# leeyevi/MV3D_TF

Measured on AMD Instinct MI355X. Metric: KITTI-shape frames/sec (RPN+3-view ROI-pool+NMS) at 1/2/4/8 MI355X, higher is better.
Workload: dtype f32

## Files before the change

### include/mv3d_hip.h

```cpp
#ifndef MV3D_HIP_H
#define MV3D_HIP_H
#include <stddef.h>
#include <stdint.h>
#ifdef __cplusplus
extern "C" {
#endif

typedef enum {
    MV3D_OK = 0,
    MV3D_ERR_INVALID_ARG = 1,
    MV3D_ERR_WORKSPACE = 2,
    MV3D_ERR_HIP = 3,
    MV3D_ERR_ZERO_DIVISION = 4
} mv3d_status;

int mv3d_version(void);
const char *mv3d_status_string(int status);


size_t mv3d_nms_workspace_bytes(int max_boxes);
int mv3d_nms_device(const float *dets_dev, int n, double thresh, int max_keep,
                    int32_t *keep_dev, int32_t *num_keep_dev, int32_t *status_dev,
                    void *workspace, size_t workspace_bytes, void *stream);

// ... 158 lines not shown
int mv3d_proposal_target_stage2_batch_devn(int batch, const float *const *rois_bv_dev, const float *const *rois_3d_dev,
                                           const int *num_rois_cap, const int32_t *const *num_rois_dev,
                                           const float *const *gt_bv_dev, const float *const *gt_3d_dev,
                                           const float *const *gt_corners_dev, const int *G, const float *const *calib_dev,
                                           const mv3d_proposal_target_params *params, const int32_t *const *fg_pick_dev,
                                           const int *n_fg, const int32_t *const *bg_pick_dev, const int *n_bg,
                                           float *const *rois_bv_out, float *const *rois_img_out, int32_t *const *labels_out,
                                           float *const *bbox_targets_out, float *const *rois_3d_out, float *const *rois_fv_out,
                                           void *const *workspace, const size_t *workspace_bytes, void *stream);

int mv3d_point_cloud_2_top(const float *points_dev, int num_points, float *top_dev, void *stream);

int mv3d_point_cloud_2_top_shape(double res, double zres, double side_lo, double side_hi, double fwd_lo, double fwd_hi,
                                 double height_lo, double height_hi, int *dims);
int mv3d_point_cloud_2_top_ranges(const float *points_dev, int num_points, double res, double zres, double side_lo, double side_hi,
                                  double fwd_lo, double fwd_hi, double height_lo, double height_hi, float *top_dev,
                                  int *status_dev, void *stream);

int mv3d_legacy_permutation(void *mt19937_state, int32_t n, int32_t *out);
typedef struct {
    int32_t n_fg, n_bg, n_low;
    int32_t pt_n_fg, pt_n_bg;
    int32_t reserved0;
    const uint8_t *fg_alive;
} mv3d_draw_frame;
typedef struct {
    int32_t rpn_batchsize;
    int32_t rpn_num_fg;
    int32_t rois_per_image;
    int32_t roi_fg_max;
} mv3d_draw_params;
int mv3d_draw_training_subsamples(void *mt19937_state, int batch, const mv3d_draw_frame *frames, const mv3d_draw_params *par,
                                  int32_t *lists, size_t lists_cap, int32_t *sizes, int32_t *scratch, size_t scratch_cap);

typedef struct {
    int32_t batch, H, W, num_classes;
    int32_t proposal_cap;
    int32_t anchor_cap;
    int32_t roi_cap;
    int32_t max_gt;
    mv3d_proposal_params proposal;
    mv3d_anchor_target_params anchor;
    mv3d_proposal_target_params target;
    mv3d_draw_params draw;
} mv3d_train_path_config;
typedef struct {
    float *blob_bv, *blob_img, *blob_3d;
    int32_t *num_proposals;
    void *proposal_ws; size_t proposal_ws_bytes;
    float *rpn_labels, *rpn_targets;
    float *anchors, *anchors_3d;
    int32_t *n_anchors;
    uint8_t *report; size_t report_row;
    int32_t *pt_counts;
    void *anchor_ws; size_t anchor_ws_bytes;
    void *target_ws; size_t target_ws_bytes;
    float *rois_bev, *rois_rgb, *rois_fv;
    float *rois_3d; int32_t *labels; float *bbox_targets;
    int32_t *lists; size_t lists_cap;
    uint8_t *h_report; size_t h_report_row;
    int32_t *h_pt_counts;
    int32_t *h_num_proposals;
    int32_t *h_lists;
    int32_t *h_scratch; size_t scratch_cap;
} mv3d_train_path_slot;
typedef struct mv3d_train_path mv3d_train_path;
int mv3d_train_path_create(const mv3d_train_path_config *config, int depth, const mv3d_train_path_slot *slots, int helper_thread,
                           mv3d_train_path **out);
int mv3d_train_path_configure(mv3d_train_path *path, const mv3d_train_path_config *config);
int mv3d_train_path_submit(mv3d_train_path *path, int slot, const float *prob_dev, const float *pred_dev, const float *im_info_dev,
                           const float *calib_dev, const float *const *gt_bv_dev, const float *const *gt_3d_dev,
                           const float *const *gt_corners_dev, const int *G, void *mt19937_state, void *stream);
int mv3d_train_path_finish(mv3d_train_path *path, int slot, int32_t *rows_out, int32_t *num_proposals_out, int32_t *sizes_out);
int mv3d_train_path_host_seconds(mv3d_train_path *path, double *wait_s, double *draw_s);
void mv3d_train_path_destroy(mv3d_train_path *path);

int mv3d_gt_encode(const float *box_cam_dev, const double *cos_sin_dev, int num_objects, const float *inv_rot_dev,
                   const float *tr_velo_to_cam_dev, float *corners_cam_dev, float *corners_lidar_dev,
                   float *boxes_3d_dev, float *boxes_bv_dev, void *stream);

int mv3d_box_detect_tail(const float *rois_3d_dev, const float *bbox_pred_dev, int num_rois, int num_classes,
                         float *corners_dev, float *pred_cnr_r_dev, float *pred_bv_dev, float *pred_bv_r_dev,
                         void *stream);

typedef struct {
    int32_t num_classes;
    int32_t rows_per_frame;
    int32_t max_per_image;
    int32_t nms_strict_gt;
    float score_thresh;
    int32_t reserved0;
    double nms_thresh;
} mv3d_detect_post_params;

size_t mv3d_detect_post_workspace_bytes(int batch, const mv3d_detect_post_params *p);
int mv3d_detect_post(const float *cls_prob_dev, const float *pred_bv_dev, const float *corners_dev,
                     const float *pred_cnr_r_dev, const int32_t *num_rois_dev, int batch,
                     const mv3d_detect_post_params *p, float *det_bv_dev, float *det_cnr_dev, float *det_cnr_r_dev,
                     int32_t *det_row_dev, int32_t *det_count_dev, int32_t *status_dev, void *workspace,
                     size_t workspace_bytes, void *stream);

size_t mv3d_loss_workspace_bytes(int rows);
int mv3d_rpn_loss(const float *rpn_cls_score_dev, const float *rpn_labels_dev, const float *rpn_bbox_pred_dev,
                  const float *rpn_bbox_targets_dev, int num_anchors, float sigma, float *losses_dev,
                  float *d_cls_score_dev, float *d_bbox_pred_dev, void *workspace, size_t workspace_bytes, void *stream);
int mv3d_rcnn_loss(const float *cls_score_dev, const int32_t *labels_dev, const float *bbox_pred_dev,
                   const float *bbox_targets_dev, int num_rois, int num_classes, int box_dim, float sigma,
// ... 167 lines not shown
```

### mv3d_tf_amd/_lib.py

```python
import ctypes as C
import os

import torch

_HERE = os.path.dirname(os.path.abspath(__file__))
LIB_PATH = os.path.join(_HERE, "libmv3d_hip.so")

OK, ERR_INVALID_ARG, ERR_WORKSPACE, ERR_HIP, ERR_ZERO_DIVISION = 0, 1, 2, 3, 4


class ProposalParams(C.Structure):
    _fields_ = [("feat_stride", C.c_int32), ("pre_nms_topN", C.c_int32), ("post_nms_topN", C.c_int32),
                ("img_height", C.c_int32), ("img_width", C.c_int32), ("img_padding", C.c_int32),
                ("nms_strict_gt", C.c_int32), ("reserved0", C.c_int32), ("nms_thresh", C.c_double), ("min_size", C.c_double)]


class DetectPostParams(C.Structure):
    _fields_ = [("num_classes", C.c_int32), ("rows_per_frame", C.c_int32), ("max_per_image", C.c_int32),
                ("nms_strict_gt", C.c_int32), ("score_thresh", C.c_float), ("reserved0", C.c_int32), ("nms_thresh", C.c_double)]


class AnchorTargetParams(C.Structure):
    _fields_ = [("feat_stride", C.c_int32), ("clobber_positives", C.c_int32),
                ("negative_overlap", C.c_double), ("positive_overlap", C.c_double)]
# ... 127 lines not shown
    "mv3d_proposal_target_stage1_batch_devn": (C.c_int, [C.c_int, _P, _P, _P, _P, _P, _P, _P, _P, _P, _P, _P, _P]),
    "mv3d_proposal_target_stage2_batch_devn": (C.c_int, [C.c_int, _P, _P, _P, _P, _P, _P, _P, _P, _P, _P, _P, _P, _P, _P, _P, _P, _P, _P,
                                                         _P, _P, _P, _P, _P]),
    "mv3d_proposal_target_workspace_bytes": (C.c_size_t, [C.c_int, C.c_int]),
    "mv3d_proposal_target_stage1": (C.c_int, [_P, _P, C.c_int, _P, _P, C.c_int, C.POINTER(ProposalTargetParams), _P, _P,
                                              C.c_size_t, _P]),
    "mv3d_proposal_target_stage2": (C.c_int, [_P, _P, C.c_int, _P, _P, _P, C.c_int, _P, C.POINTER(ProposalTargetParams),
                                              _P, C.c_int, _P, C.c_int, _P, _P, _P, _P, _P, _P, C.c_size_t, _P]),
    "mv3d_point_cloud_2_top": (C.c_int, [_P, C.c_int, _P, _P]),
    "mv3d_point_cloud_2_top_shape": (C.c_int, [C.c_double] * 8 + [_P]),
    "mv3d_point_cloud_2_top_ranges": (C.c_int, [_P, C.c_int] + [C.c_double] * 8 + [_P, _P, _P]),
    "mv3d_box_detect_tail": (C.c_int, [_P, _P, C.c_int, C.c_int, _P, _P, _P, _P, _P]),
    "mv3d_detect_post_workspace_bytes": (C.c_size_t, [C.c_int, C.POINTER(DetectPostParams)]),
    "mv3d_detect_post": (C.c_int, [_P, _P, _P, _P, _P, C.c_int, C.POINTER(DetectPostParams), _P, _P, _P, _P, _P, _P, _P, C.c_size_t,
                                   _P]),
    "mv3d_loss_workspace_bytes": (C.c_size_t, [C.c_int]),
    "mv3d_rpn_loss": (C.c_int, [_P, _P, _P, _P, C.c_int, C.c_float, _P, _P, _P, _P, C.c_size_t, _P]),
    "mv3d_rcnn_loss": (C.c_int, [_P, _P, _P, _P, C.c_int, C.c_int, C.c_int, C.c_float, _P, _P, _P, _P, C.c_size_t, _P]),
    "mv3d_roi_pool_forward_views": (C.c_int, [C.c_int, C.POINTER(RoiView), C.c_int, C.c_int, _P]),
    "mv3d_roi_pool_forward_views_cold": (C.c_int, [C.c_int, C.POINTER(RoiView), C.c_int, C.c_int, _P]),
    "mv3d_roi_pool_forward_views_half": (C.c_int, [C.c_int, C.POINTER(RoiView), C.c_int, C.c_int, C.c_int, C.c_int, _P]),
    "mv3d_roi_pool_backward_workspace_bytes": (C.c_size_t, [C.c_int, C.POINTER(RoiGradView), C.c_int, C.c_int]),
    "mv3d_roi_pool_backward_views": (C.c_int, [C.c_int, C.POINTER(RoiGradView), C.c_int, C.c_int, _P, C.c_size_t, _P]),
    "mv3d_roi_pool_pair_workspace_bytes": (C.c_size_t, [C.c_int, C.POINTER(RoiGradView), C.c_int, C.c_int]),
    "mv3d_roi_pool_forward_views_pair": (C.c_int, [C.c_int, C.POINTER(RoiView), C.c_int, C.c_int, C.c_int, _P]),
    "mv3d_roi_pool_backward_views_pair": (C.c_int, [C.c_int, C.POINTER(RoiGradView), C.c_int, C.c_int, _P, C.c_size_t, _P]),
    "mv3d_roi_pool_argmax_decode": (C.c_int, [C.c_int, C.POINTER(RoiView), C.c_int, C.c_int, C.POINTER(C.c_void_p), _P]),
    "mv3d_ROIPoolForwardLaucher": (C.c_int, [_P, C.c_float, C.c_int, C.c_int, C.c_int, C.c_int, C.c_int, C.c_int, _P, _P, _P, _P]),
    "mv3d_ROIPoolBackwardLaucher": (C.c_int, [_P, C.c_float, C.c_int, C.c_int, C.c_int, C.c_int, C.c_int, C.c_int, C.c_int, _P, _P, _P, _P]),
    "mv3d_rois_3d_to_fv": (C.c_int, [_P, C.c_int, _P, _P]),
    "mv3d_legacy_permutation": (C.c_int, [_P, C.c_int32, _P]),
    "mv3d_draw_training_subsamples": (C.c_int, [_P, C.c_int, C.POINTER(DrawFrame), C.POINTER(DrawParams), _P, C.c_size_t, _P, _P,
                                                C.c_size_t]),
    "mv3d_train_path_create": (C.c_int, [C.POINTER(TrainPathConfig), C.c_int, C.POINTER(TrainPathSlot), C.c_int, C.POINTER(C.c_void_p)]),
    "mv3d_train_path_configure": (C.c_int, [_P, C.POINTER(TrainPathConfig)]),
    "mv3d_train_path_submit": (C.c_int, [_P, C.c_int, _P, _P, _P, _P, _P, _P, _P, _P, _P, _P]),
    "mv3d_train_path_finish": (C.c_int, [_P, C.c_int, _P, _P, _P]),
    "mv3d_train_path_host_seconds": (C.c_int, [_P, C.POINTER(C.c_double), C.POINTER(C.c_double)]),
    "mv3d_train_path_destroy": (None, [_P]),
    "mv3d_gt_encode": (C.c_int, [_P, _P, C.c_int, _P, _P, _P, _P, _P, _P, _P]),
    "mv3d_conv3x3_f16": (C.c_int, [_P, _P, _P, _P, C.c_int, C.c_int, C.c_int, C.c_int, C.c_int, C.c_int, C.c_int, C.c_int, _P]),
    "mv3d_conv3x3_f32": (C.c_int, [_P, _P, _P, _P, C.c_int, C.c_int, C.c_int, C.c_int, C.c_int, C.c_int, C.c_int, _P]),
    "mv3d_maxpool2x2_f32": (C.c_int, [_P, _P, C.c_int, C.c_int, C.c_int, C.c_int, _P]),
    "mv3d_frame_nhwc_f32": (C.c_int, [_P, _P, C.c_int, C.c_int, C.c_int, C.c_int, C.c_int, _P]),
    "mv3d_conv3x3_bf16": (C.c_int, [_P, _P, _P, _P, C.c_int, C.c_int, C.c_int, C.c_int, C.c_int, C.c_int, C.c_int, C.c_int, _P]),
    "mv3d_maxpool2x2_bf16": (C.c_int, [_P, _P, C.c_int, C.c_int, C.c_int, C.c_int, _P]),
    "mv3d_frame_nhwc_bf16": (C.c_int, [_P, _P, C.c_int, C.c_int, C.c_int, C.c_int, C.c_int, _P]),
    "mv3d_conv3x3_wgrad_workspace_bytes": (C.c_size_t, [C.c_int, C.c_int, C.c_int, C.c_int, C.c_int]),
    "mv3d_conv3x3_wgrad_bf16": (C.c_int, [_P, _P, _P, _P, C.c_int, C.c_int, C.c_int, C.c_int, C.c_int, C.c_int, _P, C.c_size_t, _P]),
    "mv3d_conv3x3_wgrad_f32_workspace_bytes": (C.c_size_t, [C.c_int, C.c_int, C.c_int, C.c_int, C.c_int]),
    "mv3d_conv3x3_wgrad_f32": (C.c_int, [_P, _P, _P, _P, C.c_int, C.c_int, C.c_int, C.c_int, C.c_int, C.c_int, _P, C.c_size_t, _P]),
    "mv3d_conv3x3_pack_bf16": (C.c_int, [_P, _P, _P, C.c_int, C.c_int, C.c_int, _P]),
    "mv3d_conv3x3_gated_bf16": (C.c_int, [_P, _P, _P, _P, _P, C.c_int, C.c_int, C.c_int, C.c_int, C.c_int, _P]),
    "mv3d_maxpool2x2_bwd_f32": (C.c_int, [_P, _P, _P, C.c_int, C.c_int, C.c_int, C.c_int, _P]),
    "mv3d_maxpool2x2_bwd_bf16": (C.c_int, [_P, _P, _P, C.c_int, C.c_int, C.c_int, C.c_int, _P]),
    "mv3d_conv3x3_views_f16": (C.c_int, [C.c_int, C.POINTER(ConvView), C.c_int, C.c_int, C.c_int, C.c_int, C.c_int, _P]),
    "mv3d_conv3x3_views_bf16": (C.c_int, [C.c_int, C.POINTER(ConvView), C.c_int, C.c_int, C.c_int, C.c_int, C.c_int, _P]),
    "mv3d_conv3x3_views_f32": (C.c_int, [C.c_int, C.POINTER(ConvView), C.c_int, C.c_int, C.c_int, C.c_int, _P]),
    "mv3d_conv3x3_pool_views_f16": (C.c_int, [C.c_int, C.POINTER(ConvView), C.c_int, C.c_int, _P]),
    "mv3d_conv3x3_pool_views_bf16": (C.c_int, [C.c_int, C.POINTER(ConvView), C.c_int, C.c_int, _P]),
    "mv3d_maxpool2x2_views_f16": (C.c_int, [C.c_int, C.POINTER(PoolView), C.c_int, _P]),
    "mv3d_maxpool2x2_views_bf16": (C.c_int, [C.c_int, C.POINTER(PoolView), C.c_int, _P]),
    "mv3d_maxpool2x2_views_f32": (C.c_int, [C.c_int, C.POINTER(PoolView), C.c_int, _P]),
    "mv3d_maxpool2x2_bwd_views_bf16": (C.c_int, [C.c_int, C.POINTER(PoolView), C.c_int, _P]),
    "mv3d_maxpool2x2_bwd_views_f32": (C.c_int, [C.c_int, C.POINTER(PoolView), C.c_int, _P]),
    "mv3d_conv3x3_wgrad_views_workspace_bytes": (C.c_size_t, [C.c_int, C.POINTER(WgradView), C.c_int, C.c_int, C.c_int]),
    "mv3d_conv3x3_wgrad_views_bf16": (C.c_int, [C.c_int, C.POINTER(WgradView), C.c_int, C.c_int, C.c_int, _P, C.c_size_t, _P]),
    "mv3d_conv3x3_wgrad_views_f32": (C.c_int, [C.c_int, C.POINTER(WgradView), C.c_int, C.c_int, C.c_int, _P, C.c_size_t, _P]),
    "mv3d_conv3x3_pack_many_bf16": (C.c_int, [C.c_int, C.POINTER(PackItem), _P]),
    "mv3d_conv3x3_pack_many_f32": (C.c_int, [C.c_int, C.POINTER(PackItem), _P]),
    "mv3d_maxpool2x2_f16": (C.c_int, [_P, _P, C.c_int, C.c_int, C.c_int, C.c_int, _P]),
# ... 51 lines not shown
```

### mv3d_tf_amd/csrc/legacy_rng.hip

```cpp
#include <stdint.h>
#include <string.h>
#include "../../include/mv3d_hip.h"

namespace {

constexpr int MT_N = 624, MT_M = 397;
struct MtState { uint32_t key[MT_N]; int pos; };

inline void mt_gen(MtState *s)
{
    uint32_t *k = s->key;
    int i;
    for (i = 0; i < MT_N - MT_M; ++i) {
        const uint32_t y = (k[i] & 0x80000000u) | (k[i + 1] & 0x7fffffffu);
        k[i] = k[i + MT_M] ^ (y >> 1) ^ ((y & 1u) ? 0x9908b0dfu : 0u);
    }
    for (; i < MT_N - 1; ++i) {
        const uint32_t y = (k[i] & 0x80000000u) | (k[i + 1] & 0x7fffffffu);
        k[i] = k[i + (MT_M - MT_N)] ^ (y >> 1) ^ ((y & 1u) ? 0x9908b0dfu : 0u);
    }
    const uint32_t y = (k[MT_N - 1] & 0x80000000u) | (k[0] & 0x7fffffffu);
    k[MT_N - 1] = k[MT_M - 1] ^ (y >> 1) ^ ((y & 1u) ? 0x9908b0dfu : 0u);
    s->pos = 0;
}

inline uint32_t mt_next(MtState *s)
{
    if (s->pos == MT_N) mt_gen(s);
    uint32_t y = s->key[s->pos++];
    y ^= (y >> 11);
    y ^= (y << 7) & 0x9d2c5680u;
    y ^= (y << 15) & 0xefc60000u;
    y ^= (y >> 18);
    return y;
}

void permutation(MtState *s, int32_t n, int32_t *x)
{
    for (int32_t i = 0; i < n; ++i) x[i] = i;
    int32_t i = n - 1;
    int pos = s->pos;
    uint32_t t[MT_N];
    int t_lo = MT_N;
    while (i >= 1) {
        const uint32_t mask = 0xffffffffu >> __builtin_clz((uint32_t)i);
        const int32_t lo = (int32_t)(mask >> 1);
        while (i > lo) {
            if (pos == MT_N) { mt_gen(s); pos = 0; t_lo = MT_N; }
            if (t_lo > pos) {
                for (int k = pos; k < MT_N; ++k) {
                    uint32_t y = s->key[k];
                    y ^= (y >> 11);
                    y ^= (y << 7) & 0x9d2c5680u;
                    y ^= (y << 15) & 0xefc60000u;
                    y ^= (y >> 18);
                    t[k] = y;
                }
                t_lo = pos;
            }
            while (pos < MT_N && i > lo) {
                const uint32_t j = t[pos++] & mask;
                const bool ok = j <= (uint32_t)i;
                const uint32_t jj = ok ? j : (uint32_t)i;
                const int32_t a = x[i], b = x[jj];
                x[i] = b; x[jj] = a;
                i -= ok ? 1 : 0;
            }
        }
    }
    s->pos = pos;
}

}

extern "C" int mv3d_legacy_permutation(void *mt19937_state, int32_t n, int32_t *out)
{
    if (!mt19937_state || n < 0 || (n > 0 && !out)) return MV3D_ERR_INVALID_ARG;
    MtState *s = (MtState *)mt19937_state;
    if (s->pos < 0 || s->pos > MT_N) return MV3D_ERR_INVALID_ARG;
    permutation(s, n, out);
    return MV3D_OK;
}

extern "C" int mv3d_draw_training_subsamples(void *mt19937_state, int batch, const mv3d_draw_frame *frames,
                                             const mv3d_draw_params *par, int32_t *lists, size_t lists_cap, int32_t *sizes,
                                             int32_t *scratch, size_t scratch_cap)
{
    if (!mt19937_state || batch <= 0 || !frames || !par || !lists || !sizes || !scratch) return MV3D_ERR_INVALID_ARG;
    MtState *s = (MtState *)mt19937_state;
    if (s->pos < 0 || s->pos > MT_N) return MV3D_ERR_INVALID_ARG;
    size_t o = 0;
    auto emit = [&](int32_t n, int32_t take, bool draw, int32_t *size_out) -> bool {
        *size_out = 0;
        if (!draw) return true;
        if (n < 0 || (size_t)n > scratch_cap || take < 0 || take > n || o + (size_t)take > lists_cap) return false;
        if (take == n) {
            permutation(s, n, lists + o);
        } else {
            permutation(s, n, scratch);
            memcpy(lists + o, scratch, (size_t)take * sizeof(int32_t));
        }
        *size_out = take;
        o += (size_t)take;
        return true;
    };
    for (int b = 0; b < batch; ++b) {
        const mv3d_draw_frame &f = frames[b];
        int32_t *sz = sizes + 5 * b;
        if (f.n_fg < 0 || f.n_bg < 0 || f.n_low < 0 || f.pt_n_fg < 0 || f.pt_n_bg < 0 || (f.n_fg > 0 && !f.fg_alive))
            return MV3D_ERR_INVALID_ARG;
        const int32_t num_fg = par->rpn_num_fg;
        const int32_t *dis_fg = lists + o;
        if (!emit(f.n_fg, f.n_fg - num_fg, f.n_fg > num_fg, &sz[0])) return MV3D_ERR_WORKSPACE;
        const int32_t num_bg = par->rpn_batchsize - (f.n_fg < num_fg ? f.n_fg : num_fg);
        if (!emit(f.n_bg, f.n_bg - num_bg, f.n_bg > num_bg, &sz[1])) return MV3D_ERR_WORKSPACE;
        int32_t n_pos = 0;
        if (f.n_fg > 0) {
            if ((size_t)f.n_fg > scratch_cap) return MV3D_ERR_WORKSPACE;
            uint8_t *alive = (uint8_t *)scratch;
            for (int32_t i = 0; i < f.n_fg; ++i) alive[i] = f.fg_alive[i] ? 1 : 0;
            for (int32_t i = 0; i < sz[0]; ++i) alive[dis_fg[i]] = 0;
            for (int32_t i = 0; i < f.n_fg; ++i) n_pos += alive[i];
        }
        const int32_t num_bg2 = par->rpn_batchsize - n_pos;
        if (!emit(f.n_low, f.n_low - num_bg2, f.n_low > num_bg2, &sz[2])) return MV3D_ERR_WORKSPACE;
        const int32_t fg_n = par->roi_fg_max < f.pt_n_fg ? par->roi_fg_max : f.pt_n_fg;
        if (!emit(f.pt_n_fg, fg_n, f.pt_n_fg > 0, &sz[3])) return MV3D_ERR_WORKSPACE;
        const int32_t bg_room = par->rois_per_image - fg_n;
        const int32_t bg_n = bg_room < f.pt_n_bg ? bg_room : f.pt_n_bg;
        if (!emit(f.pt_n_bg, bg_n < 0 ? 0 : bg_n, f.pt_n_bg > 0, &sz[4])) return MV3D_ERR_WORKSPACE;
    }
    return MV3D_OK;
}
```

### mv3d_tf_amd/csrc/train_stream.hip

```cpp
#include <hip/hip_runtime.h>
#include <chrono>
#include <condition_variable>
#include <deque>
#include <mutex>
#include <new>
#include <thread>
#include <vector>
#include "common.h"
#include "../../include/mv3d_hip.h"

#define TP_MAX_BATCH 16

namespace {

enum SlotState { TP_IDLE = 0, TP_SUBMITTED = 1, TP_STAGED = 2 };

struct Slot {
    mv3d_train_path_slot buf;
    hipEvent_t ev = nullptr;
    int state = TP_IDLE, rc = MV3D_OK;
    hipStream_t stream = nullptr;
    void *mt = nullptr;
    const float *calib = nullptr;
    const float *gt_bv[TP_MAX_BATCH], *gt_3d[TP_MAX_BATCH], *gt_c[TP_MAX_BATCH];
// ... 14 lines not shown
{
#ifdef MV3D_TUNING
    return getenv("MV3D_TRAIN_PATH_COPIES") != nullptr;
#else
    return false;
#endif
}

__global__ __launch_bounds__(256) void tp_report_kernel(const uint8_t *__restrict__ report, size_t report_row, uint8_t *__restrict__ h_report,
                                                        size_t h_row, int B, const int32_t *__restrict__ pt_counts, int32_t *__restrict__ h_pt,
                                                        const int32_t *__restrict__ nump, int32_t *__restrict__ h_nump)
{
    const size_t v = h_row / 16;
    for (size_t i = threadIdx.x; i < (size_t)B * v; i += 256) {
        const size_t b = i / v, j = i - b * v;
        reinterpret_cast<uint4 *>(h_report + b * h_row)[j] = reinterpret_cast<const uint4 *>(report + b * report_row)[j];
    }
    for (int i = threadIdx.x; i < 4 * B; i += 256) h_pt[i] = pt_counts[i];
    for (int i = threadIdx.x; i < 2 * B; i += 256) h_nump[i] = nump[i];
}

}

struct mv3d_train_path {
    mv3d_train_path_config cfg;
    mv3d_proposal_target_params tpar[TP_MAX_BATCH];
    int depth = 0, device = 0;
    std::vector<Slot> slots;
    bool threaded = false, stop = false;
    std::thread helper;
    std::mutex m;
    std::condition_variable cv_work, cv_done;
    std::deque<int> queue;
    double t_wait = 0.0, t_draw = 0.0;
};

namespace {

bool config_ok(const mv3d_train_path_config &c)
{
    return c.batch >= 1 && c.batch <= TP_MAX_BATCH && c.H > 0 && c.W > 0 && c.num_classes >= 1 && c.proposal_cap > 0 && c.anchor_cap > 0 &&
           c.roi_cap > 0 && c.max_gt > 0 && c.draw.rois_per_image <= c.roi_cap;
}

void set_params(mv3d_train_path *tp, const mv3d_train_path_config &c)
{
    tp->cfg = c;
    for (int b = 0; b < c.batch; ++b) {
        tp->tpar[b] = c.target;
        tp->tpar[b].num_classes = c.num_classes;
        tp->tpar[b].frame_index = b;
    }
}

bool slot_ok(const mv3d_train_path_config &c, const mv3d_train_path_slot &s)
{
    const size_t N = (size_t)4 * c.H * c.W, B = (size_t)c.batch;
    if (!s.blob_bv || !s.blob_img || !s.blob_3d || !s.num_proposals || !s.proposal_ws || !s.rpn_labels || !s.rpn_targets || !s.anchors ||
        !s.anchors_3d || !s.n_anchors || !s.report || !s.pt_counts || !s.anchor_ws || !s.target_ws || !s.rois_bev || !s.rois_rgb ||
        !s.rois_3d || !s.labels || !s.bbox_targets || !s.lists || !s.h_report || !s.h_pt_counts || !s.h_num_proposals || !s.h_lists ||
        !s.h_scratch)
        return false;
    if (s.report_row % MV3D_ALIGN || s.report_row < 32 + N || s.h_report_row < 32 || s.h_report_row > s.report_row) return false;
    if (s.anchor_ws_bytes % MV3D_ALIGN || s.target_ws_bytes % MV3D_ALIGN) return false;
    if (s.lists_cap < B * (3 * N + 2 * ((size_t)c.proposal_cap + c.max_gt))) return false;
    if (s.scratch_cap < (N > (size_t)c.proposal_cap + c.max_gt ? N : (size_t)c.proposal_cap + c.max_gt)) return false;
    return true;
// ... 18 lines not shown

#define TP_HIP(expr)                                 \
    do {                                             \
        if ((expr) != hipSuccess) return MV3D_ERR_HIP; \
    } while (0)

int host_stage(mv3d_train_path *tp, Slot &s)
{
    const mv3d_train_path_config &c = tp->cfg;
    const mv3d_train_path_slot &u = s.buf;
    const int B = c.batch, H = c.H, W = c.W;
    const auto t0 = std::chrono::steady_clock::now();
    TP_HIP(hipEventSynchronize(s.ev));
    const auto t1 = std::chrono::steady_clock::now();
    for (int b = 0; b < B; ++b)
        if (u.h_num_proposals[B + b] & MV3D_FLAG_ZERO_DIVISION) return MV3D_ERR_ZERO_DIVISION;
    mv3d_draw_frame fr[TP_MAX_BATCH];
    for (int b = 0; b < B; ++b) {
        const uint8_t *head = u.h_report + (size_t)b * u.h_report_row;
        const int32_t *cnt = (const int32_t *)head;
        fr[b].n_fg = cnt[1]; fr[b].n_bg = cnt[2]; fr[b].n_low = cnt[3];
        fr[b].pt_n_fg = u.h_pt_counts[4 * b + 1]; fr[b].pt_n_bg = u.h_pt_counts[4 * b + 2];
        fr[b].reserved0 = 0;
        if (cnt[1] < 0 || (size_t)cnt[1] > (size_t)4 * H * W) return MV3D_ERR_INVALID_ARG;
        if (32 + (size_t)cnt[1] <= u.h_report_row) {
            fr[b].fg_alive = head + 32;
        } else {
            s.spill[b].resize((size_t)cnt[1]);
            TP_HIP(hipMemcpyAsync(s.spill[b].data(), s.a_fgh[b], (size_t)cnt[1], hipMemcpyDeviceToHost, s.stream));
            TP_HIP(hipStreamSynchronize(s.stream));
            fr[b].fg_alive = s.spill[b].data();
        }
    }
    int rc = mv3d_draw_training_subsamples(s.mt, B, fr, &c.draw, u.h_lists, u.lists_cap, s.sizes, u.h_scratch, u.scratch_cap);
    const auto t2 = std::chrono::steady_clock::now();
    {
        std::lock_guard<std::mutex> g(tp->m);
        tp->t_wait += std::chrono::duration<double>(t1 - t0).count();
        tp->t_draw += std::chrono::duration<double>(t2 - t1).count();
    }
    if (rc != MV3D_OK) return rc;
    size_t off[5 * TP_MAX_BATCH + 1];
    off[0] = 0;
    for (int k = 0; k < 5 * B; ++k) off[k + 1] = off[k] + (size_t)s.sizes[k];
    const int32_t *const lists = u.lists;
    if (off[5 * B]) TP_HIP(hipMemcpyAsync(u.lists, u.h_lists, off[5 * B] * sizeof(int32_t), hipMemcpyHostToDevice, s.stream));
    const int32_t *lst[5][TP_MAX_BATCH];
    int cnt[5][TP_MAX_BATCH];
    for (int b = 0; b < B; ++b)
        for (int k = 0; k < 5; ++k) {
            cnt[k][b] = s.sizes[5 * b + k];
            lst[k][b] = cnt[k][b] ? lists + off[5 * b + k] : nullptr;
        }
    rc = mv3d_anchor_target_stage2_batch(B, H, W, &c.anchor, lst[0], cnt[0], lst[1], cnt[1], lst[2], cnt[2], u.rpn_labels, u.anchors,
                                         u.anchors_3d, u.n_anchors, c.anchor_cap, s.a_ws, u.anchor_ws_bytes, s.stream);
    if (rc != MV3D_OK) return rc;
    float *o_bev[TP_MAX_BATCH], *o_rgb[TP_MAX_BATCH], *o_fv[TP_MAX_BATCH], *o_3d[TP_MAX_BATCH], *o_tg[TP_MAX_BATCH];
    int32_t *o_lab[TP_MAX_BATCH];
    const float *cal[TP_MAX_BATCH];
    size_t row = 0;
    for (int b = 0; b < B; ++b) {
        const int S = cnt[3][b] + cnt[4][b];
        s.rows[b] = S;
        if (row + (size_t)S > (size_t)B * c.roi_cap) return MV3D_ERR_WORKSPACE;
        o_bev[b] = S ? u.rois_bev + row * 5 : nullptr;
        o_rgb[b] = S ? u.rois_rgb + row * 5 : nullptr;
        o_fv[b] = (S && u.rois_fv) ? u.rois_fv + row * 5 : nullptr;
        o_3d[b] = S ? u.rois_3d + row * 7 : nullptr;
        o_lab[b] = S ? u.labels + row : nullptr;
        o_tg[b] = S ? u.bbox_targets + row * 24 * c.num_classes : nullptr;
        cal[b] = s.calib + (size_t)b * 48;
        row += (size_t)S;
    }
    return mv3d_proposal_target_stage2_batch_devn(B, s.p_bv, s.p_3d, s.p_cap, s.p_num, s.gt_bv, s.gt_3d, s.gt_c, s.G, cal, tp->tpar, lst[3],
                                                  cnt[3], lst[4], cnt[4], o_bev, o_rgb, o_lab, o_tg, o_3d, u.rois_fv ? o_fv : nullptr, s.p_ws,
                                                  s.p_wsz, s.stream);
}

int host_stage_noexcept(mv3d_train_path *tp, Slot &s)
{
    try {
        return host_stage(tp, s);
    } catch (...) {
        return MV3D_ERR_WORKSPACE;
    }
}

void helper_main(mv3d_train_path *tp)
{
    (void)hipSetDevice(tp->device);
    for (;;) {
        int k;
        {
            std::unique_lock<std::mutex> g(tp->m);
            tp->cv_work.wait(g, [&] { return tp->stop || !tp->queue.empty(); });
            if (tp->queue.empty()) return;
            k = tp->queue.front();
            tp->queue.pop_front();
        }
        Slot &s = tp->slots[k];
        const int rc = host_stage_noexcept(tp, s);
        {
            std::lock_guard<std::mutex> g(tp->m);
            s.rc = rc;
            s.state = TP_STAGED;
        }
        tp->cv_done.notify_all();
    }
}

}

extern "C" int mv3d_train_path_create(const mv3d_train_path_config *config, int depth, const mv3d_train_path_slot *slots, int helper_thread,
                                      mv3d_train_path **out)
{
    if (!config || !slots || !out || depth < 1 || depth > 64 || !config_ok(*config)) return MV3D_ERR_INVALID_ARG;
    for (int k = 0; k < depth; ++k)
        if (!slot_ok(*config, slots[k])) return MV3D_ERR_INVALID_ARG;
    mv3d_train_path *tp = new (std::nothrow) mv3d_train_path();
    if (!tp) return MV3D_ERR_HIP;
    set_params(tp, *config);
    tp->depth = depth;
    if (hipGetDevice(&tp->device) != hipSuccess) { delete tp; return MV3D_ERR_HIP; }
    try {
        tp->slots.resize((size_t)depth);
    } catch (...) {
        delete tp;
        return MV3D_ERR_HIP;
// ... 111 lines not shown
    if (tp->threaded) {
        std::unique_lock<std::mutex> g(tp->m);
        if (s.state == TP_IDLE) return MV3D_ERR_INVALID_ARG;
        tp->cv_done.wait(g, [&] { return s.state == TP_STAGED; });
        rc = s.rc;
    } else {
        {
            std::lock_guard<std::mutex> g(tp->m);
            if (s.state != TP_SUBMITTED) return MV3D_ERR_INVALID_ARG;
        }
        rc = host_stage_noexcept(tp, s);
    }
    const int B = tp->cfg.batch;
    if (rc == MV3D_OK) {
        for (int b = 0; b < B; ++b) { rows_out[b] = s.rows[b]; num_proposals_out[b] = s.buf.h_num_proposals[b]; }
        if (sizes_out)
            for (int k = 0; k < 5 * B; ++k) sizes_out[k] = s.sizes[k];
    }
    std::lock_guard<std::mutex> g(tp->m);
    s.state = TP_IDLE;
    return rc;
}

extern "C" int mv3d_train_path_host_seconds(mv3d_train_path *tp, double *wait_s, double *draw_s)
{
    if (!tp) return MV3D_ERR_INVALID_ARG;
    std::lock_guard<std::mutex> g(tp->m);
    if (wait_s) *wait_s = tp->t_wait;
    if (draw_s) *draw_s = tp->t_draw;
    tp->t_wait = tp->t_draw = 0.0;
    return MV3D_OK;
}

extern "C" void mv3d_train_path_destroy(mv3d_train_path *tp)
{
    if (!tp) return;
    if (tp->threaded) {
        {
            std::lock_guard<std::mutex> g(tp->m);
            tp->stop = true;
        }
        tp->cv_work.notify_all();
        tp->helper.join();
    }
    for (Slot &s : tp->slots)
        if (s.ev) (void)hipEventDestroy(s.ev);
    delete tp;
}
```

### mv3d_tf_amd/train_path.py

```python
import ctypes as C

import numpy as np
import numpy.random as npr
import torch

from . import ops
from ._lib import AnchorTargetParams, DrawParams, ProposalTargetParams, TrainPathConfig, TrainPathSlot, check, lib
from .fast_rcnn.config import cfg

_HEAD = 4096


def draw_subsamples_host(head, n_fg_flags_fetch, N):
    T = cfg.TRAIN
    n_inside, n_fg, n_bg, n_low = (int(v) for v in head[:16].view(np.int32))
    num_fg = int(T.RPN_FG_FRACTION * T.RPN_BATCHSIZE)
    dis_fg = npr.permutation(n_fg)[:n_fg - num_fg] if n_fg > num_fg else None
    num_bg = T.RPN_BATCHSIZE - min(n_fg, num_fg)
    dis_bg1 = npr.permutation(n_bg)[:n_bg - num_bg] if n_bg > num_bg else None
    n_pos = 0
    if n_fg:
        alive = (head[32:32 + n_fg] if 32 + n_fg <= len(head) else n_fg_flags_fetch()[:n_fg]).astype(bool)
        if dis_fg is not None:
            alive[dis_fg] = False
# ... 131 lines not shown
            check(L.mv3d_train_path_configure(self._h, C.byref(conf)), "mv3d_train_path_configure")
            self._cfg_key, self._config = key, conf
        self._next = (self._next + 1) % len(self.slots)
        if s.stream is not None:
            s.stream.wait_stream(torch.cuda.current_stream())
        st = (s.stream or torch.cuda.current_stream()).cuda_stream
        s.inputs = (prob, pred, im_info, calib, gt)
        s.G = G
        mt = _global_mt19937_address()
        PP = C.c_void_p * B
        check(L.mv3d_train_path_submit(self._h, s.index, prob.data_ptr(), pred.data_ptr(), im_info.data_ptr(), calib.data_ptr(),
                                       PP(*[g[0].data_ptr() for g in gt]), PP(*[g[1].data_ptr() for g in gt]),
                                       PP(*[g[2].data_ptr() for g in gt]), (C.c_int * B)(*G), mt, st), "mv3d_train_path_submit")
        s.busy = True
        return s

    def close(self):
        h, self._h = getattr(self, "_h", None), None
        if h:
            lib().mv3d_train_path_destroy(h)

    def __del__(self):
        try:
            self.close()
        except Exception:
            pass

    @property
    def host_seconds(self):
        w, d = C.c_double(), C.c_double()
        check(lib().mv3d_train_path_host_seconds(self._h, C.byref(w), C.byref(d)), "mv3d_train_path_host_seconds")
        return w.value, d.value

    def finish(self, s):
        s.busy = False
        check(lib().mv3d_train_path_finish(self._h, s.index, s.rows_c, s.nprop_c, s.sizes_c), "mv3d_train_path_finish")
        S = list(s.rows_c)
        St = sum(S)
        return {"rpn_labels": s.rpn_labels, "rpn_targets": s.rpn_targets, "anchors": s.anchors, "anchors_3d": s.anchors_3d,
                "n_anchors": s.n_anchors, "rois": {k: v[:St] for k, v in s.rois.items()}, "rois_3d": s.rois_3d[:St],
                "labels": s.labels[:St], "bbox_targets": s.bbox_targets[:St], "S": S,
                "num_proposals": list(s.nprop_c), "proposals": s.prop, "stream": s.stream, "draw_sizes": list(s.sizes_c)}
```

Before: 16890.

## Draw RPN subsample discard sets with sparse partial shuffle and AVX2 skip-ahead

Result: no change. 16750 (-0.8%).

```diff
diff --git a/include/mv3d_hip.h b/include/mv3d_hip.h
--- a/include/mv3d_hip.h
+++ b/include/mv3d_hip.h
@@ -214,6 +214,8 @@
 } mv3d_draw_params;
 int mv3d_draw_training_subsamples(void *mt19937_state, int batch, const mv3d_draw_frame *frames, const mv3d_draw_params *par,
                                   int32_t *lists, size_t lists_cap, int32_t *sizes, int32_t *scratch, size_t scratch_cap);
+int mv3d_draw_training_subsets(void *mt19937_state, int batch, const mv3d_draw_frame *frames, const mv3d_draw_params *par,
+                               int32_t *lists, size_t lists_cap, int32_t *sizes, int32_t *scratch, size_t scratch_cap, int flags);
 
 typedef struct {
     int32_t batch, H, W, num_classes;
@@ -255,6 +257,7 @@
                            const float *const *gt_corners_dev, const int *G, void *mt19937_state, void *stream);
 int mv3d_train_path_finish(mv3d_train_path *path, int slot, int32_t *rows_out, int32_t *num_proposals_out, int32_t *sizes_out);
 int mv3d_train_path_host_seconds(mv3d_train_path *path, double *wait_s, double *draw_s);
+int mv3d_train_path_host_profile(mv3d_train_path *path, double *out);
 void mv3d_train_path_destroy(mv3d_train_path *path);
 
 int mv3d_gt_encode(const float *box_cam_dev, const double *cos_sin_dev, int num_objects, const float *inv_rot_dev,
diff --git a/mv3d_tf_amd/_lib.py b/mv3d_tf_amd/_lib.py
--- a/mv3d_tf_amd/_lib.py
+++ b/mv3d_tf_amd/_lib.py
@@ -183,11 +183,14 @@
     "mv3d_legacy_permutation": (C.c_int, [_P, C.c_int32, _P]),
     "mv3d_draw_training_subsamples": (C.c_int, [_P, C.c_int, C.POINTER(DrawFrame), C.POINTER(DrawParams), _P, C.c_size_t, _P, _P,
                                                 C.c_size_t]),
+    "mv3d_draw_training_subsets": (C.c_int, [_P, C.c_int, C.POINTER(DrawFrame), C.POINTER(DrawParams), _P, C.c_size_t, _P, _P,
+                                             C.c_size_t, C.c_int]),
     "mv3d_train_path_create": (C.c_int, [C.POINTER(TrainPathConfig), C.c_int, C.POINTER(TrainPathSlot), C.c_int, C.POINTER(C.c_void_p)]),
     "mv3d_train_path_configure": (C.c_int, [_P, C.POINTER(TrainPathConfig)]),
     "mv3d_train_path_submit": (C.c_int, [_P, C.c_int, _P, _P, _P, _P, _P, _P, _P, _P, _P, _P]),
     "mv3d_train_path_finish": (C.c_int, [_P, C.c_int, _P, _P, _P]),
     "mv3d_train_path_host_seconds": (C.c_int, [_P, C.POINTER(C.c_double), C.POINTER(C.c_double)]),
+    "mv3d_train_path_host_profile": (C.c_int, [_P, C.POINTER(C.c_double)]),
     "mv3d_train_path_destroy": (None, [_P]),
     "mv3d_gt_encode": (C.c_int, [_P, _P, C.c_int, _P, _P, _P, _P, _P, _P, _P]),
     "mv3d_conv3x3_f16": (C.c_int, [_P, _P, _P, _P, C.c_int, C.c_int, C.c_int, C.c_int, C.c_int, C.c_int, C.c_int, C.c_int, _P]),
diff --git a/mv3d_tf_amd/csrc/legacy_rng.hip b/mv3d_tf_amd/csrc/legacy_rng.hip
--- a/mv3d_tf_amd/csrc/legacy_rng.hip
+++ b/mv3d_tf_amd/csrc/legacy_rng.hip
@@ -1,74 +1,46 @@
 #include <stdint.h>
 #include <string.h>
 #include "../../include/mv3d_hip.h"
+
+#if defined(__x86_64__) && !defined(__HIP_DEVICE_COMPILE__)
+#define MV3D_RNG_X86 1
+#include <immintrin.h>
+#endif
 
 namespace {
 
 constexpr int MT_N = 624, MT_M = 397;
 struct MtState { uint32_t key[MT_N]; int pos; };
 
-inline void mt_gen(MtState *s)
-{
-    uint32_t *k = s->key;
-    int i;
-    for (i = 0; i < MT_N - MT_M; ++i) {
-        const uint32_t y = (k[i] & 0x80000000u) | (k[i + 1] & 0x7fffffffu);
-        k[i] = k[i + MT_M] ^ (y >> 1) ^ ((y & 1u) ? 0x9908b0dfu : 0u);
-    }
-    for (; i < MT_N - 1; ++i) {
-        const uint32_t y = (k[i] & 0x80000000u) | (k[i + 1] & 0x7fffffffu);
-        k[i] = k[i + (MT_M - MT_N)] ^ (y >> 1) ^ ((y & 1u) ? 0x9908b0dfu : 0u);
-    }
-    const uint32_t y = (k[MT_N - 1] & 0x80000000u) | (k[0] & 0x7fffffffu);
-    k[MT_N - 1] = k[MT_M - 1] ^ (y >> 1) ^ ((y & 1u) ? 0x9908b0dfu : 0u);
-    s->pos = 0;
+constexpr int SET_BLOCK = 16;
+constexpr int32_t SET_MAX_KEEP = 1024;
+constexpr int SET_TABLE_LOG2 = 11, SET_TABLE = 1 << SET_TABLE_LOG2;
+constexpr int32_t SET_MIN_N = 1024, SET_MIN_N_PER_KEEP = 32;
+
 }
 
-inline uint32_t mt_next(MtState *s)
+namespace {
+#define MV3D_RNG_NS rng_portable
+#include "legacy_rng_body.h"
+#undef MV3D_RNG_NS
+#ifdef MV3D_RNG_X86
+#pragma clang attribute push(__attribute__((target("avx2,popcnt"))), apply_to = function)
+#define MV3D_RNG_NS rng_avx2
+#define MV3D_RNG_AVX2 1
+#include "legacy_rng_body.h"
+#undef MV3D_RNG_AVX2
+#undef MV3D_RNG_NS
+#pragma clang attribute pop
+#endif
+
+bool have_avx2()
 {
-    if (s->pos == MT_N) mt_gen(s);
-    uint32_t y = s->key[s->pos++];
-    y ^= (y >> 11);
-    y ^= (y << 7) & 0x9d2c5680u;
-    y ^= (y << 15) & 0xefc60000u;
-    y ^= (y >> 18);
-    return y;
-}
-
-void permutation(MtState *s, int32_t n, int32_t *x)
-{
-    for (int32_t i = 0; i < n; ++i) x[i] = i;
-    int32_t i = n - 1;
-    int pos = s->pos;
-    uint32_t t[MT_N];
-    int t_lo = MT_N;
-    while (i >= 1) {
-        const uint32_t mask = 0xffffffffu >> __builtin_clz((uint32_t)i);
-        const int32_t lo = (int32_t)(mask >> 1);
-        while (i > lo) {
-            if (pos == MT_N) { mt_gen(s); pos = 0; t_lo = MT_N; }
-            if (t_lo > pos) {
-                for (int k = pos; k < MT_N; ++k) {
-                    uint32_t y = s->key[k];
-                    y ^= (y >> 11);
-                    y ^= (y << 7) & 0x9d2c5680u;
-                    y ^= (y << 15) & 0xefc60000u;
-                    y ^= (y >> 18);
-                    t[k] = y;
-                }
-                t_lo = pos;
-            }
-            while (pos < MT_N && i > lo) {
-                const uint32_t j = t[pos++] & mask;
-                const bool ok = j <= (uint32_t)i;
-                const uint32_t jj = ok ? j : (uint32_t)i;
-                const int32_t a = x[i], b = x[jj];
-                x[i] = b; x[jj] = a;
-                i -= ok ? 1 : 0;
-            }
-        }
-    }
-    s->pos = pos;
+#ifdef MV3D_RNG_X86
+    static const bool yes = __builtin_cpu_supports("avx2") && __builtin_cpu_supports("popcnt");
+    return yes;
+#else
+    return false;
+#endif
 }
 
 }
@@ -78,7 +50,7 @@
     if (!mt19937_state || n < 0 || (n > 0 && !out)) return MV3D_ERR_INVALID_ARG;
     MtState *s = (MtState *)mt19937_state;
     if (s->pos < 0 || s->pos > MT_N) return MV3D_ERR_INVALID_ARG;
-    permutation(s, n, out);
+    rng_portable::permutation(s, n, out);
     return MV3D_OK;
 }
 
@@ -89,46 +61,24 @@
     if (!mt19937_state || batch <= 0 || !frames || !par || !lists || !sizes || !scratch) return MV3D_ERR_INVALID_ARG;
     MtState *s = (MtState *)mt19937_state;
     if (s->pos < 0 || s->pos > MT_N) return MV3D_ERR_INVALID_ARG;
-    size_t o = 0;
-    auto emit = [&](int32_t n, int32_t take, bool draw, int32_t *size_out) -> bool {
-        *size_out = 0;
-        if (!draw) return true;
-        if (n < 0 || (size_t)n > scratch_cap || take < 0 || take > n || o + (size_t)take > lists_cap) return false;
-        if (take == n) {
-            permutation(s, n, lists + o);
-        } else {
-            permutation(s, n, scratch);
-            memcpy(lists + o, scratch, (size_t)take * sizeof(int32_t));
-        }
-        *size_out = take;
-        o += (size_t)take;
-        return true;
-    };
-    for (int b = 0; b < batch; ++b) {
-        const mv3d_draw_frame &f = frames[b];
-        int32_t *sz = sizes + 5 * b;
-        if (f.n_fg < 0 || f.n_bg < 0 || f.n_low < 0 || f.pt_n_fg < 0 || f.pt_n_bg < 0 || (f.n_fg > 0 && !f.fg_alive))
-            return MV3D_ERR_INVALID_ARG;
-        const int32_t num_fg = par->rpn_num_fg;
-        const int32_t *dis_fg = lists + o;
-        if (!emit(f.n_fg, f.n_fg - num_fg, f.n_fg > num_fg, &sz[0])) return MV3D_ERR_WORKSPACE;
-        const int32_t num_bg = par->rpn_batchsize - (f.n_fg < num_fg ? f.n_fg : num_fg);
-        if (!emit(f.n_bg, f.n_bg - num_bg, f.n_bg > num_bg, &sz[1])) return MV3D_ERR_WORKSPACE;
-        int32_t n_pos = 0;
-        if (f.n_fg > 0) {
-            if ((size_t)f.n_fg > scratch_cap) return MV3D_ERR_WORKSPACE;
-            uint8_t *alive = (uint8_t *)scratch;
-            for (int32_t i = 0; i < f.n_fg; ++i) alive[i] = f.fg_alive[i] ? 1 : 0;
-            for (int32_t i = 0; i < sz[0]; ++i) alive[dis_fg[i]] = 0;
-            for (int32_t i = 0; i < f.n_fg; ++i) n_pos += alive[i];
-        }
-        const int32_t num_bg2 = par->rpn_batchsize - n_pos;
-        if (!emit(f.n_low, f.n_low - num_bg2, f.n_low > num_bg2, &sz[2])) return MV3D_ERR_WORKSPACE;
-        const int32_t fg_n = par->roi_fg_max < f.pt_n_fg ? par->roi_fg_max : f.pt_n_fg;
-        if (!emit(f.pt_n_fg, fg_n, f.pt_n_fg > 0, &sz[3])) return MV3D_ERR_WORKSPACE;
-        const int32_t bg_room = par->rois_per_image - fg_n;
-        const int32_t bg_n = bg_room < f.pt_n_bg ? bg_room : f.pt_n_bg;
-        if (!emit(f.pt_n_bg, bg_n < 0 ? 0 : bg_n, f.pt_n_bg > 0, &sz[4])) return MV3D_ERR_WORKSPACE;
+    rng_portable::Drawer d = {s, lists, lists_cap, 0, scratch, scratch_cap, false, false};
+    return d.batch(batch, frames, par, sizes);
+}
+
+extern "C" int mv3d_draw_training_subsets(void *mt19937_state, int batch, const mv3d_draw_frame *frames,
+                                          const mv3d_draw_params *par, int32_t *lists, size_t lists_cap, int32_t *sizes,
+                                          int32_t *scratch, size_t scratch_cap, int flags)
+{
+    if (!mt19937_state || batch <= 0 || !frames || !par || !lists || !sizes || !scratch || (flags & ~3)) return MV3D_ERR_INVALID_ARG;
+    MtState *s = (MtState *)mt19937_state;
+    if (s->pos < 0 || s->pos > MT_N) return MV3D_ERR_INVALID_ARG;
+    const bool every_n = (flags & 2) != 0;
+#ifdef MV3D_RNG_X86
+    if (!(flags & 1) && have_avx2()) {
+        rng_avx2::Drawer d = {s, lists, lists_cap, 0, scratch, scratch_cap, true, every_n};
+        return d.batch(batch, frames, par, sizes);
     }
-    return MV3D_OK;
+#endif
+    rng_portable::Drawer d = {s, lists, lists_cap, 0, scratch, scratch_cap, true, every_n};
+    return d.batch(batch, frames, par, sizes);
 }
diff --git a/mv3d_tf_amd/csrc/legacy_rng_body.h b/mv3d_tf_amd/csrc/legacy_rng_body.h
--- /dev/null
+++ b/mv3d_tf_amd/csrc/legacy_rng_body.h
@@ -0,0 +1,223 @@
+namespace MV3D_RNG_NS {
+
+inline void mt_chunk(uint32_t *__restrict dst, const uint32_t *__restrict src, int count)
+{
+    for (int i = 0; i < count; ++i) {
+        const uint32_t y = (dst[i] & 0x80000000u) | (dst[i + 1] & 0x7fffffffu);
+        dst[i] = src[i] ^ (y >> 1) ^ ((y & 1u) ? 0x9908b0dfu : 0u);
+    }
+}
+
+inline void mt_gen(MtState *s)
+{
+    uint32_t *k = s->key;
+    mt_chunk(k, k + MT_M, MT_N - MT_M);
+    mt_chunk(k + (MT_N - MT_M), k, MT_N - MT_M);
+    mt_chunk(k + 2 * (MT_N - MT_M), k + (MT_N - MT_M), MT_N - 1 - 2 * (MT_N - MT_M));
+    const uint32_t y = (k[MT_N - 1] & 0x80000000u) | (k[0] & 0x7fffffffu);
+    k[MT_N - 1] = k[MT_M - 1] ^ (y >> 1) ^ ((y & 1u) ? 0x9908b0dfu : 0u);
+    s->pos = 0;
+}
+
+inline void mt_temper(const MtState *s, int pos, uint32_t *t)
+{
+    for (int k = pos; k < MT_N; ++k) {
+        uint32_t y = s->key[k];
+        y ^= (y >> 11);
+        y ^= (y << 7) & 0x9d2c5680u;
+        y ^= (y << 15) & 0xefc60000u;
+        y ^= (y >> 18);
+        t[k] = y;
+    }
+}
+
+void permutation(MtState *s, int32_t n, int32_t *x)
+{
+    for (int32_t i = 0; i < n; ++i) x[i] = i;
+    int32_t i = n - 1;
+    int pos = s->pos;
+    uint32_t t[MT_N];
+    int t_lo = MT_N;
+    while (i >= 1) {
+        const uint32_t mask = 0xffffffffu >> __builtin_clz((uint32_t)i);
+        const int32_t lo = (int32_t)(mask >> 1);
+        while (i > lo) {
+            if (pos == MT_N) { mt_gen(s); pos = 0; t_lo = MT_N; }
+            if (t_lo > pos) {
+                mt_temper(s, pos, t);
+                t_lo = pos;
+            }
+            while (pos < MT_N && i > lo) {
+                const uint32_t j = t[pos++] & mask;
+                const bool ok = j <= (uint32_t)i;
+                const uint32_t jj = ok ? j : (uint32_t)i;
+                const int32_t a = x[i], b = x[jj];
+                x[i] = b; x[jj] = a;
+                i -= ok ? 1 : 0;
+            }
+        }
+    }
+    s->pos = pos;
+}
+
+template <int W>
+inline void count_le2(const uint32_t *t, uint32_t mask, int32_t a, int32_t b, int *n_a, int *n_b)
+{
+#ifdef MV3D_RNG_AVX2
+    const __m256i m = _mm256_set1_epi32((int)mask), va = _mm256_set1_epi32(a), vb = _mm256_set1_epi32(b);
+    uint64_t gt_a = 0, gt_b = 0;
+    for (int k = 0; k < W; k += 8) {
+        const __m256i v = _mm256_and_si256(_mm256_loadu_si256((const __m256i *)(t + k)), m);
+        gt_a |= (uint64_t)(unsigned)_mm256_movemask_ps(_mm256_castsi256_ps(_mm256_cmpgt_epi32(v, va))) << k;
+        gt_b |= (uint64_t)(unsigned)_mm256_movemask_ps(_mm256_castsi256_ps(_mm256_cmpgt_epi32(v, vb))) << k;
+    }
+    *n_a = W - __builtin_popcountll(gt_a);
+    *n_b = W - __builtin_popcountll(gt_b);
+#else
+    int ca = 0, cb = 0;
+    for (int k = 0; k < W; ++k) {
+        const int32_t v = (int32_t)(t[k] & mask);
+        ca += v <= a ? 1 : 0;
+        cb += v <= b ? 1 : 0;
+    }
+    *n_a = ca; *n_b = cb;
+#endif
+}
+
+template <int W>
+inline int32_t set_advance(const uint32_t *t, uint32_t mask, int32_t i)
+{
+    int sure, maybe;
+    count_le2<W>(t, mask, i - W, i, &sure, &maybe);
+    if (sure == maybe) return i - sure;
+    if constexpr (W > SET_BLOCK) {
+        return set_advance<W / 2>(t + W / 2, mask, set_advance<W / 2>(t, mask, i));
+    } else {
+        for (int k = 0; k < W; ++k) i -= (int32_t)(t[k] & mask) <= i ? 1 : 0;
+        return i;
+    }
+}
+
+inline int set_slot(const int32_t *key, int32_t p)
+{
+    int h = (int)(((uint32_t)p * 2654435761u) >> (32 - SET_TABLE_LOG2));
+    while (key[h] != -1 && key[h] != p) h = (h + 1) & (SET_TABLE - 1);
+    return h;
+}
+
+void permutation_head_set(MtState *s, int32_t n, int32_t keep, int32_t *out, uint32_t *bits)
+{
+    int pos = s->pos;
+    uint32_t t[MT_N];
+    int t_lo = MT_N;
+    int32_t i = n - 1;
+    const int32_t stop = n - keep;
+    const int32_t words = (n + 31) / 32;
+    for (int32_t w = 0; w < words; ++w) bits[w] = 0;
+    int32_t key[SET_TABLE], val[SET_TABLE];
+    for (int k = 0; k < SET_TABLE; ++k) key[k] = -1;
+    while (i >= stop) {
+        const uint32_t mask = 0xffffffffu >> __builtin_clz((uint32_t)i);
+        const int32_t lo = (int32_t)(mask >> 1);
+        while (i > lo && i >= stop) {
+            if (pos == MT_N) { mt_gen(s); pos = 0; t_lo = MT_N; }
+            if (t_lo > pos) { mt_temper(s, pos, t); t_lo = pos; }
+            const int32_t j = (int32_t)(t[pos++] & mask);
+            if (j > i) continue;
+            const int hi = set_slot(key, i);
+            const int32_t vi = key[hi] == i ? val[hi] : i;
+            const int hj = set_slot(key, j);
+            const int32_t vj = key[hj] == j ? val[hj] : j;
+            bits[vj >> 5] |= 1u << (vj & 31);
+            key[hj] = j; val[hj] = vi;
+            --i;
+        }
+    }
+    while (i >= 1) {
+        const uint32_t mask = 0xffffffffu >> __builtin_clz((uint32_t)i);
+        const int32_t lo = (int32_t)(mask >> 1);
+        while (i > lo) {
+            if (pos == MT_N) { mt_gen(s); pos = 0; t_lo = MT_N; }
+            if (t_lo > pos) { mt_temper(s, pos, t); t_lo = pos; }
+            if (mask >= 16 * SET_BLOCK * SET_BLOCK * 4 - 1)
+                for (; pos + 4 * SET_BLOCK <= MT_N && i - 4 * SET_BLOCK > lo; pos += 4 * SET_BLOCK) i = set_advance<4 * SET_BLOCK>(t + pos, mask, i);
+            if (mask >= 4 * SET_BLOCK * SET_BLOCK * 4 - 1)
+                for (; pos + 2 * SET_BLOCK <= MT_N && i - 2 * SET_BLOCK > lo; pos += 2 * SET_BLOCK) i = set_advance<2 * SET_BLOCK>(t + pos, mask, i);
+            if (mask >= SET_BLOCK * SET_BLOCK * 4 - 1)
+                for (; pos + SET_BLOCK <= MT_N && i - SET_BLOCK > lo; pos += SET_BLOCK) i = set_advance<SET_BLOCK>(t + pos, mask, i);
+            while (pos < MT_N && i > lo) i -= (int32_t)(t[pos++] & mask) <= i ? 1 : 0;
+        }
+    }
+    s->pos = pos;
+    int32_t o = 0, next = 0;
+    for (int32_t w = 0; w < words; ++w) {
+        uint32_t b = bits[w];
+        while (b) {
+            const int32_t kv = 32 * w + __builtin_ctz(b);
+            b &= b - 1;
+            for (int32_t v = next; v < kv; ++v) out[o++] = v;
+            next = kv + 1;
+        }
+    }
+    for (int32_t v = next; v < n; ++v) out[o++] = v;
+}
+
+struct Drawer {
+    MtState *s;
+    int32_t *lists;
+    size_t lists_cap, o;
+    int32_t *scratch;
+    size_t scratch_cap;
+    bool sets, every_n;
+
+    bool emit(int32_t n, int32_t take, bool draw, bool as_set, int32_t *size_out)
+    {
+        *size_out = 0;
+        if (!draw) return true;
+        if (n < 0 || (size_t)n > scratch_cap || take < 0 || take > n || o + (size_t)take > lists_cap) return false;
+        if (as_set && take >= 1 && n - take >= 1 && n - take <= SET_MAX_KEEP && (every_n || take >= SET_MIN_N + (SET_MIN_N_PER_KEEP - 1) * (n - take))) {
+            permutation_head_set(s, n, n - take, lists + o, (uint32_t *)scratch);
+        } else if (take == n) {
+            permutation(s, n, lists + o);
+        } else {
+            permutation(s, n, scratch);
+            memcpy(lists + o, scratch, (size_t)take * sizeof(int32_t));
+        }
+        *size_out = take;
+        o += (size_t)take;
+        return true;
+    }
+
+    int batch(int batch, const mv3d_draw_frame *frames, const mv3d_draw_params *par, int32_t *sizes)
+    {
+        for (int b = 0; b < batch; ++b) {
+            const mv3d_draw_frame &f = frames[b];
+            int32_t *sz = sizes + 5 * b;
+            if (f.n_fg < 0 || f.n_bg < 0 || f.n_low < 0 || f.pt_n_fg < 0 || f.pt_n_bg < 0 || (f.n_fg > 0 && !f.fg_alive))
+                return MV3D_ERR_INVALID_ARG;
+            const int32_t num_fg = par->rpn_num_fg;
+            const int32_t *dis_fg = lists + o;
+            if (!emit(f.n_fg, f.n_fg - num_fg, f.n_fg > num_fg, sets, &sz[0])) return MV3D_ERR_WORKSPACE;
+            const int32_t num_bg = par->rpn_batchsize - (f.n_fg < num_fg ? f.n_fg : num_fg);
+            if (!emit(f.n_bg, f.n_bg - num_bg, f.n_bg > num_bg, sets, &sz[1])) return MV3D_ERR_WORKSPACE;
+            int32_t n_pos = 0;
+            if (f.n_fg > 0) {
+                if ((size_t)f.n_fg > scratch_cap) return MV3D_ERR_WORKSPACE;
+                uint8_t *alive = (uint8_t *)scratch;
+                for (int32_t i = 0; i < f.n_fg; ++i) alive[i] = f.fg_alive[i] ? 1 : 0;
+                for (int32_t i = 0; i < sz[0]; ++i) alive[dis_fg[i]] = 0;
+                for (int32_t i = 0; i < f.n_fg; ++i) n_pos += alive[i];
+            }
+            const int32_t num_bg2 = par->rpn_batchsize - n_pos;
+            if (!emit(f.n_low, f.n_low - num_bg2, f.n_low > num_bg2, sets, &sz[2])) return MV3D_ERR_WORKSPACE;
+            const int32_t fg_n = par->roi_fg_max < f.pt_n_fg ? par->roi_fg_max : f.pt_n_fg;
+            if (!emit(f.pt_n_fg, fg_n, f.pt_n_fg > 0, false, &sz[3])) return MV3D_ERR_WORKSPACE;
+            const int32_t bg_room = par->rois_per_image - fg_n;
+            const int32_t bg_n = bg_room < f.pt_n_bg ? bg_room : f.pt_n_bg;
+            if (!emit(f.pt_n_bg, bg_n < 0 ? 0 : bg_n, f.pt_n_bg > 0, false, &sz[4])) return MV3D_ERR_WORKSPACE;
+        }
+        return MV3D_OK;
+    }
+};
+
+}
diff --git a/mv3d_tf_amd/csrc/train_stream.hip b/mv3d_tf_amd/csrc/train_stream.hip
--- a/mv3d_tf_amd/csrc/train_stream.hip
+++ b/mv3d_tf_amd/csrc/train_stream.hip
@@ -70,7 +70,7 @@
     std::mutex m;
     std::condition_variable cv_work, cv_done;
     std::deque<int> queue;
-    double t_wait = 0.0, t_draw = 0.0;
+    double t_wait = 0.0, t_draw = 0.0, t_enqueue = 0.0, t_idle = 0.0;
 };
 
 namespace {
@@ -155,13 +155,23 @@
             fr[b].fg_alive = s.spill[b].data();
         }
     }
-    int rc = mv3d_draw_training_subsamples(s.mt, B, fr, &c.draw, u.h_lists, u.lists_cap, s.sizes, u.h_scratch, u.scratch_cap);
+    int rc = mv3d_draw_training_subsets(s.mt, B, fr, &c.draw, u.h_lists, u.lists_cap, s.sizes, u.h_scratch, u.scratch_cap, 0);
     const auto t2 = std::chrono::steady_clock::now();
     {
         std::lock_guard<std::mutex> g(tp->m);
         tp->t_wait += std::chrono::duration<double>(t1 - t0).count();
         tp->t_draw += std::chrono::duration<double>(t2 - t1).count();
     }
+    struct EnqueueTimer {
+        mv3d_train_path *tp;
+        std::chrono::steady_clock::time_point from;
+        ~EnqueueTimer()
+        {
+            const double dt = std::chrono::duration<double>(std::chrono::steady_clock::now() - from).count();
+            std::lock_guard<std::mutex> g(tp->m);
+            tp->t_enqueue += dt;
+        }
+    } enqueue_timer{tp, t2};
     if (rc != MV3D_OK) return rc;
     size_t off[5 * TP_MAX_BATCH + 1];
     off[0] = 0;
@@ -216,7 +226,9 @@
         int k;
         {
             std::unique_lock<std::mutex> g(tp->m);
+            const auto idle0 = std::chrono::steady_clock::now();
             tp->cv_work.wait(g, [&] { return tp->stop || !tp->queue.empty(); });
+            tp->t_idle += std::chrono::duration<double>(std::chrono::steady_clock::now() - idle0).count();
             if (tp->queue.empty()) return;
             k = tp->queue.front();
             tp->queue.pop_front();
@@ -394,6 +406,15 @@
     return MV3D_OK;
 }
 
+extern "C" int mv3d_train_path_host_profile(mv3d_train_path *tp, double *out)
+{
+    if (!tp || !out) return MV3D_ERR_INVALID_ARG;
+    std::lock_guard<std::mutex> g(tp->m);
+    out[0] = tp->t_wait; out[1] = tp->t_draw; out[2] = tp->t_enqueue; out[3] = tp->t_idle;
+    tp->t_wait = tp->t_draw = tp->t_enqueue = tp->t_idle = 0.0;
+    return MV3D_OK;
+}
+
 extern "C" void mv3d_train_path_destroy(mv3d_train_path *tp)
 {
     if (!tp) return;
diff --git a/mv3d_tf_amd/train_path.py b/mv3d_tf_amd/train_path.py
--- a/mv3d_tf_amd/train_path.py
+++ b/mv3d_tf_amd/train_path.py
@@ -187,6 +187,12 @@
         check(lib().mv3d_train_path_host_seconds(self._h, C.byref(w), C.byref(d)), "mv3d_train_path_host_seconds")
         return w.value, d.value
 
+    @property
+    def host_profile(self):
+        out = (C.c_double * 4)()
+        check(lib().mv3d_train_path_host_profile(self._h, out), "mv3d_train_path_host_profile")
+        return dict(zip(("wait", "draw", "enqueue", "idle"), out))
+
     def finish(self, s):
         s.busy = False
         check(lib().mv3d_train_path_finish(self._h, s.index, s.rows_c, s.nprop_c, s.sizes_c), "mv3d_train_path_finish")
```
